# sb-ai-lab/RePlay

Hardware: NVIDIA H100
Metric: sasrec_train_seq_per_s (higher is better)
Workload: dtype bf16

## Files before the change

### replay_b200/csrc/rp_ce_head.cu

```cuda
#include <type_traits>

#include "rp_host.h"
#include "rp_gemm_desc.h"
#include "rp_sm90.cuh"

namespace rp {

static constexpr int kT = 128;
static constexpr int kChunk = 128 * 128;
static constexpr float kLog2e = 1.4426950408889634f;
static constexpr float kLn2 = 0.6931471805599453f;
static constexpr int kThreads = 256;
static constexpr int kTN = 64;

__device__ __forceinline__ float bce_sigmoid(float x, float& one_plus_e) {
  const float e = ex2f(-fabsf(x) * kLog2e);
  one_plus_e = 1.f + e;
  return __fdividef(x >= 0.f ? 1.f : e, one_plus_e);
}
template <int KCH, int NSTAGE, bool BCE = false>
__global__ void __launch_bounds__(kThreads, 1)
ce_fwd_kernel(const __grid_constant__ CUtensorMap tmA, const __grid_constant__ CUtensorMap tmB,
              const int32_t* __restrict__ n_valid_ptr, int n_items, int n_splits, const float* __restrict__ bias,
              float2* __restrict__ part ,
// ... 219 lines not shown
    for (int i = 0; i < (int)gridDim.x; ++i) s += reinterpret_cast<volatile float*>(block_sums)[i];
    loss_out[0] = s * inv_n;
    loss_out[1] = inv_n;
  }
}

struct CeDirect {
  __nv_bfloat16* d_hc;
  float* lse;
  float* cvec;
  float* row_loss;
  CeRowOpts row;
  int use_lse_off;
};

__device__ __forceinline__ float crow_of(const CeDirect& d, int r, int n_valid) {
  return r < n_valid ? (d.use_lse_off ? -d.lse[r] * kLog2e : 0.f) : -INFINITY;
}

__global__ void __launch_bounds__(1024) ce_loss_reduce_kernel(const float* __restrict__ row_loss, const int32_t* __restrict__ n_valid_ptr,
                                                              const int32_t* __restrict__ safe_flag, float* __restrict__ loss_out,
                                                              int run_if_safe) {
  if (safe_flag && (*safe_flag != 0) != (run_if_safe != 0)) return;
  __shared__ float red[1024];
  const int n_valid = *n_valid_ptr;
  float a = 0.f;
  for (int i = threadIdx.x; i < n_valid; i += 1024) a += row_loss[i];
  red[threadIdx.x] = a;
  __syncthreads();
  for (int o = 512; o > 0; o >>= 1) {
    if ((int)threadIdx.x < o) red[threadIdx.x] += red[threadIdx.x + o];
    __syncthreads();
  }
  if (threadIdx.x == 0) {
    const float inv_n = n_valid > 0 ? 1.f / (float)n_valid : 0.f;
    loss_out[0] = red[0] * inv_n;
    loss_out[1] = inv_n;
  }
}

template <int KCH, int NSTAGE, int TN, int MODE, bool HAS_BIAS>
__global__ void __launch_bounds__(kThreads, 1)
ce_bwd_kernel(const __grid_constant__ CUtensorMap tmA, const __grid_constant__ CUtensorMap tmB,
              const __nv_bfloat16* __restrict__ a_rows ,
              const float* __restrict__ cvec , const int32_t* __restrict__ labels,
              const __nv_bfloat16* __restrict__ table, const float* __restrict__ loss_inv ,
              const int32_t* __restrict__ n_valid_ptr, int n_items, const float* __restrict__ bias,
              float* __restrict__ d_bias, void* __restrict__ out, const int32_t* __restrict__ safe_flag, int run_if_safe,
              int n_splits, int capacity, float* __restrict__ zpart, const CeDirect direct) {
  constexpr bool BCE = (MODE >= 3);
  constexpr bool COLCONST = (MODE == 1 || MODE == 4);
  constexpr bool FUSED = (MODE == 2 || MODE == 3);
  constexpr int D = KCH * 64;
  constexpr int kChunkB = TN * 128;
  constexpr int kStage = KCH * kChunkB;
  constexpr int PITCH = D + 4;
  constexpr int kSlots = 2, DW = D / kSlots;
  if (safe_flag && (*safe_flag != 0) != (run_if_safe != 0)) return;
  extern __shared__ __align__(1024) uint8_t smem_raw[];
  uint8_t* smem = reinterpret_cast<uint8_t*>((reinterpret_cast<uintptr_t>(smem_raw) + 1023) & ~uintptr_t(1023));
  uint8_t* sA = smem;
  uint8_t* sB = smem + KCH * kChunk;
  __shared__ float s_row[kT];
  __shared__ float s_dot[kSlots][kT];
  __shared__ uint64_t bar_a, bar_full[NSTAGE];
  __shared__ uint32_t s_released[NSTAGE];

  const int lane = threadIdx.x & 31;
  const int n_valid = *n_valid_ptr;
  const int split = FUSED ? blockIdx.x % n_splits : 0;
  const int n_rows = COLCONST ? n_items : n_valid;
  const int n_cols = COLCONST ? n_valid : n_items;
  const int n_grid = (n_cols + kTN - 1) / kTN;
  const int row_tile = FUSED ? blockIdx.x / n_splits : blockIdx.x;
  const int c_begin = FUSED ? (int)(((long long)n_grid * split) / n_splits) * kTN : 0;
  const int c_end = FUSED ? min(n_cols, (int)(((long long)n_grid * (split + 1)) / n_splits) * kTN) : n_cols;
  const int n_ct = c_end > c_begin ? (c_end - c_begin + TN - 1) / TN : 0;
  const int r0 = row_tile * kT;
  if (r0 >= n_rows) return;

  if (threadIdx.x == 0) {
    mbar_init(&bar_a, 1);
    for (int i = 0; i < NSTAGE; ++i) {
      mbar_init(&bar_full[i], 1);
      s_released[i] = 0;
    }
    fence_barrier_init();
    tma_prefetch_desc(&tmA);
    tma_prefetch_desc(&tmB);
  }
  __syncthreads();
  auto issue = [&](int jl) {
    const uint32_t s = jl % NSTAGE;
    mbar_arrive_expect_tx(&bar_full[s], kStage);
    for (int kc = 0; kc < KCH; ++kc) tma_load_2d(sB + s * kStage + kc * kChunkB, &tmB, &bar_full[s], kc * 64, c_begin + jl * TN);
  };
  if (threadIdx.x == 0) {
    mbar_arrive_expect_tx(&bar_a, KCH * kChunk);
    for (int kc = 0; kc < KCH; ++kc) tma_load_2d(sA + kc * kChunk, &tmA, &bar_a, kc * 64, r0);
    for (int jl = 0; jl < NSTAGE && jl < n_ct; ++jl) issue(jl);
  }
  const int t = threadIdx.x & 127, wg = threadIdx.x >> 7;
  const int fc = frag_col(t);
  const int rla = 64 * wg + frag_row(t), rlb = rla + 8;
  float crow_a = 0.f, crow_b = 0.f;
  if (MODE == 0) {
    crow_a = (r0 + rla < n_valid) ? cvec[r0 + rla] : -INFINITY;
    crow_b = (r0 + rlb < n_valid) ? cvec[r0 + rlb] : -INFINITY;
  }
  if (FUSED && !BCE) {
    crow_a = (r0 + rla < n_valid) ? (direct.use_lse_off ? -direct.lse[r0 + rla] * kLog2e : 0.f) : -INFINITY;
    crow_b = (r0 + rlb < n_valid) ? (direct.use_lse_off ? -direct.lse[r0 + rlb] * kLog2e : 0.f) : -INFINITY;
  }
  float brow_a = 0.f, brow_b = 0.f;
  if (BCE && COLCONST && HAS_BIAS) {
    brow_a = r0 + rla < n_items ? __ldg(bias + r0 + rla) : 0.f;
    brow_b = r0 + rlb < n_items ? __ldg(bias + r0 + rlb) : 0.f;
  }
  float za = 0.f, zb = 0.f;
  float acc[D / 2];
  acc_zero(acc);
  float sacc[TN / 2];
  mbar_wait(&bar_a, 0);
  const uint32_t a_base = smem_u32(sA) + wg * 8192;
  auto issue_s = [&](int jl) {
    mbar_wait(&bar_full[jl % NSTAGE], (jl / NSTAGE) & 1);
    const uint32_t b0 = smem_u32(sB + (jl % NSTAGE) * kStage);
    wg_fence();
#pragma unroll
    for (int kc = 0; kc < KCH; ++kc)
#pragma unroll
      for (int ks = 0; ks < 4; ++ks)
        WgmmaSS<TN>::template run<0, 0>(sacc, desc_k(a_base + kc * kChunk + ks * 32), desc_k(b0 + kc * kChunkB + ks * 32),
                                        (kc | ks) != 0);
    wg_commit();
  };
  constexpr bool kSAhead = MODE != 3;
  if (n_ct > 0) {
    issue_s(0);
    wg_wait<0>();
    wg_fence_acc(sacc);
  }
  if (kSAhead && wg == 1 && n_ct > 0) named_bar_arrive(2, 256);
  for (int jl = 0; jl < n_ct; ++jl) {
    const uint32_t s = jl % NSTAGE;
    const uint32_t b0 = smem_u32(sB + s * kStage);
    const int col0 = c_begin + jl * TN + fc;
    uint32_t pk[TN / 4];
    if constexpr (BCE) {
      float pa = 1.f, pb = 1.f;
#pragma unroll
      for (int q = 0; q < TN / 8; ++q) {
        float g[4];
#pragma unroll
        for (int e = 0; e < 2; ++e) {
          const int col = col0 + 8 * q + e;
          const bool in = col < c_end;
          float va = sacc[4 * q + e], vb = sacc[4 * q + 2 + e];
          if (HAS_BIAS) {
            const float ba = COLCONST ? brow_a : (in ? __ldg(bias + col) : 0.f);
            const float bb = COLCONST ? brow_b : ba;
            va += ba;
// ... 18 lines not shown
        pk[2 * q + 1] = pack_bf16(g[2], g[3]);
      }
      if (FUSED) {
        za += __log2f(pa) * kLn2;
        zb += __log2f(pb) * kLn2;
      }
    } else {
#pragma unroll
      for (int q = 0; q < TN / 8; ++q) {
        float g[4];
#pragma unroll
        for (int e = 0; e < 2; ++e) {
          const int col = col0 + 8 * q + e;
          float va = sacc[4 * q + e], vb = sacc[4 * q + 2 + e];
          if (COLCONST) {
            const float cc = __ldg(cvec + col);
            g[e] = ex2f(fmaf(va, kLog2e, cc));
            g[2 + e] = ex2f(fmaf(vb, kLog2e, cc));
          } else {
            const bool in = col < c_end;
            if (HAS_BIAS && in) {
              const float bb = __ldg(bias + col);
              va += bb;
              vb += bb;
            }
            g[e] = in ? ex2f(fmaf(va, kLog2e, crow_a)) : 0.f;
            g[2 + e] = in ? ex2f(fmaf(vb, kLog2e, crow_b)) : 0.f;
          }
        }
        if (FUSED || (COLCONST && HAS_BIAS)) {
          za += g[0] + g[1];
// ... 1 lines not shown
        }
        pk[2 * q] = pack_bf16(g[0], g[1]);
        pk[2 * q + 1] = pack_bf16(g[2], g[3]);
      }
    }
    if (kSAhead) named_bar_sync(2 + wg, 256);
    wg_fence();
#pragma unroll
    for (int kk = 0; kk < TN / 16; ++kk) {
      const uint32_t af[4] = {pk[4 * kk], pk[4 * kk + 1], pk[4 * kk + 2], pk[4 * kk + 3]};
      WgmmaRS<D>::template run<1>(acc, af, desc_mn(b0 + kk * 2048, kChunkB), 1);
    }
    wg_commit();
    const bool more = jl + 1 < n_ct;
    if constexpr (kSAhead) {
      if (more) issue_s(jl + 1);
      else wg_commit();
      if (wg == 0) named_bar_arrive(3, 256);
      else if (more) named_bar_arrive(2, 256);
      wg_wait<1>();
    } else {
      wg_wait<0>();
    }
    wg_fence_acc(acc);
    __syncwarp();
    if (lane == 0 && jl + NSTAGE < n_ct && smem_count_acq_rel(&s_released[s]) % 8 == 7) {
      fence_proxy_async();
      issue(jl + NSTAGE);
    }
    if (!kSAhead && more) issue_s(jl + 1);
    wg_wait<0>();
    wg_fence_acc(sacc);
  }
#pragma unroll
  for (int o = 1; o <= 2; o <<= 1) {
    za += __shfl_xor_sync(0xffffffffu, za, o);
    zb += __shfl_xor_sync(0xffffffffu, zb, o);
  }
  if (fc == 0) {
    s_row[rla] = za;
    s_row[rlb] = zb;
  }
  named_bar_sync(1, 256);
  float* stage = reinterpret_cast<float*>(sB);
  acc_to_stage(acc, stage, PITCH, 64 * wg, 0);
  named_bar_sync(1, 256);
  const int row = t, slot = wg;
  const int r = r0 + row;
  const float* arow = stage + row * PITCH + slot * DW;
  if constexpr (BCE) {
    const float inv_n = n_valid > 0 ? 1.f / (float)n_valid : 0.f;
    if (COLCONST) {
      if (r < n_items) {
// ... 44 lines not shown
#pragma unroll 4
        for (int c = 0; c < DW; c += 4) dst[c >> 2] = *reinterpret_cast<const float4*>(arow + c);
      }
    }
  } else if (COLCONST) {
    float* o = reinterpret_cast<float*>(out);
    const float rs = (HAS_BIAS && r < n_items) ? __expf(bias[r]) : 1.f;
    if (HAS_BIAS && slot == 0 && r < n_items) d_bias[r] = s_row[row] * rs;
    if (r < n_items) {
      float4* dst = reinterpret_cast<float4*>(o + (size_t)r * D + slot * DW);
#pragma unroll 4
      for (int c = 0; c < DW; c += 4) {
        const float4 v = *reinterpret_cast<const float4*>(arow + c);
        dst[c >> 2] = make_float4(v.x * rs, v.y * rs, v.z * rs, v.w * rs);
      }
    }
  } else if (FUSED && direct.d_hc != nullptr) {
    const float z = s_row[row];
    const bool live = r < n_valid;
    const float inv_n = n_valid > 0 ? 1.f / (float)n_valid : 0.f;
    const int y = live ? labels[r] : 0;
    float wg_ = (live && direct.row.w_ext) ? direct.row.w_ext[r] : 1.f;
    if (direct.row.kind == 1) {
      float dp = 0.f;
      if (live) {
        const uint4* ey = reinterpret_cast<const uint4*>(table + (size_t)y * D + slot * DW);
        const uint4* hr = reinterpret_cast<const uint4*>(a_rows + (size_t)r * D + slot * DW);
#pragma unroll 4
        for (int q = 0; q < DW / 8; ++q) {
          const uint4 e = __ldg(ey + q), hh = __ldg(hr + q);
          const __nv_bfloat162* e2 = reinterpret_cast<const __nv_bfloat162*>(&e);
          const __nv_bfloat162* h2 = reinterpret_cast<const __nv_bfloat162*>(&hh);
#pragma unroll
          for (int pp = 0; pp < 4; ++pp) {
            const float2 ef = __bfloat1622float2(e2[pp]), hf = __bfloat1622float2(h2[pp]);
            dp = fmaf(hf.x, ef.x, fmaf(hf.y, ef.y, dp));
          }
        }
      }
      s_dot[slot][row] = dp;
      named_bar_sync(1, 256);
      float zy0 = s_dot[0][row] + s_dot[1][row];
      if (HAS_BIAS) zy0 += bias[y];
      named_bar_sync(1, 256);
      float rl_unused;
      if (live) ce_row_terms(direct.row, r, __logf(z) - crow_of(direct, r, n_valid) * kLn2, zy0, rl_unused, wg_);
    }
    const float scale = live ? wg_ * inv_n / z : 0.f;
    const float lab = wg_ * inv_n;
    float dot = 0.f;
    if (live) {
      const uint4* ey = reinterpret_cast<const uint4*>(table + (size_t)y * D + slot * DW);
      const uint4* hr = reinterpret_cast<const uint4*>(a_rows + (size_t)r * D + slot * DW);
      uint4* dst = reinterpret_cast<uint4*>(direct.d_hc + (size_t)r * D + slot * DW);
#pragma unroll 4
      for (int q = 0; q < DW / 8; ++q) {
        const uint4 e = __ldg(ey + q), hh = __ldg(hr + q);
        const __nv_bfloat162* e2 = reinterpret_cast<const __nv_bfloat162*>(&e);
        const __nv_bfloat162* h2 = reinterpret_cast<const __nv_bfloat162*>(&hh);
        uint4 w;
        uint32_t* w32 = reinterpret_cast<uint32_t*>(&w);
#pragma unroll
        for (int pp = 0; pp < 4; ++pp) {
          const float2 ef = __bfloat1622float2(e2[pp]), hf = __bfloat1622float2(h2[pp]);
          dot = fmaf(hf.x, ef.x, fmaf(hf.y, ef.y, dot));
          w32[pp] = pack_bf16(arow[8 * q + 2 * pp] * scale - lab * ef.x, arow[8 * q + 2 * pp + 1] * scale - lab * ef.y);
        }
        dst[q] = w;
      }
    }
    s_dot[slot][row] = dot;
    named_bar_sync(1, 256);
    if (slot == 0 && r < capacity) {
      if (live) {
        float zy = s_dot[0][row] + s_dot[1][row];
        if (HAS_BIAS) zy += bias[y];
        const float lse2 = log2f(z) - crow_of(direct, r, n_valid);
        float rl, wg2;
        ce_row_terms(direct.row, r, lse2 * kLn2, zy, rl, wg2);
        direct.lse[r] = lse2 * kLn2;
        direct.cvec[r] = -lse2 + log2f(wg2 * inv_n);
        direct.row_loss[r] = rl;
        if (direct.row.roww) direct.row.roww[r] = wg2;
      } else {
        direct.cvec[r] = -INFINITY;
      }
    }
  } else if (FUSED) {
    float* o = reinterpret_cast<float*>(out) + (size_t)split * capacity * D;
    if (r < n_valid) {
      if (slot == 0) zpart[(size_t)split * capacity + r] = s_row[row];
      float4* dst = reinterpret_cast<float4*>(o + (size_t)r * D + slot * DW);
#pragma unroll 4
      for (int c = 0; c < DW; c += 4) dst[c >> 2] = *reinterpret_cast<const float4*>(arow + c);
    }
  } else {
    __nv_bfloat16* o = reinterpret_cast<__nv_bfloat16*>(out);
    if (r < n_valid) {
      const float inv_n = loss_inv[0] * (direct.row.roww ? direct.row.roww[r] : 1.f);
      const int y = labels[r];
      const uint4* ey = reinterpret_cast<const uint4*>(table + (size_t)y * D + slot * DW);
      uint4* dst = reinterpret_cast<uint4*>(o + (size_t)r * D + slot * DW);
#pragma unroll 4
      for (int q = 0; q < DW / 8; ++q) {
        const uint4 e = ey[q];
        const __nv_bfloat162* e2 = reinterpret_cast<const __nv_bfloat162*>(&e);
        uint4 w;
        uint32_t* w32 = reinterpret_cast<uint32_t*>(&w);
#pragma unroll
// ... 75 lines not shown
    me = fmaxf(me, __shfl_xor_sync(0xffffffffu, me, o));
    mb = fmaxf(mb, __shfl_xor_sync(0xffffffffu, mb, o));
  }
  if (lane == 0) {
    atomicMax(bound + 0, __float_as_uint(mh));
    atomicMax(bound + 1, __float_as_uint(me));
    atomicMax(bound + 2, __float_as_uint(mb));
  }
}

__global__ void ce_flag_kernel(const unsigned int* __restrict__ bound, int32_t* __restrict__ safe_flag) {
  const float b = sqrtf(__uint_as_float(bound[0]) * __uint_as_float(bound[1])) + __uint_as_float(bound[2]);
  *safe_flag = (b * kLog2e < 100.f) ? 1 : 0;
}

__global__ void ce_fused_finalize_kernel(const float* __restrict__ part_dh, const float* __restrict__ zpart,
                                         const __nv_bfloat16* __restrict__ hc, const __nv_bfloat16* __restrict__ table,
                                         const int32_t* __restrict__ labels, const float* __restrict__ bias,
                                         const int32_t* __restrict__ n_valid_ptr, const int32_t* __restrict__ safe_flag,
                                         int n_splits, int z_slots, int capacity, int d, float* __restrict__ lse_out,
                                         float* __restrict__ cvec, __nv_bfloat16* __restrict__ d_hc,
                                         float* __restrict__ block_sums, unsigned int* __restrict__ ticket,
                                         float* __restrict__ loss_out, const CeRowOpts row, int use_lse_off, int run_if_safe) {
  if ((*safe_flag != 0) != (run_if_safe != 0)) return;
  const int n_valid = *n_valid_ptr;
  const float inv_n = n_valid > 0 ? 1.f / (float)n_valid : 0.f;
  const int lane = threadIdx.x & 31, wpb = blockDim.x >> 5;
  float local = 0.f;
  for (int t = blockIdx.x * wpb + (threadIdx.x >> 5); t < capacity; t += gridDim.x * wpb) {
    if (t >= n_valid) {
      if (lane == 0) cvec[t] = -INFINITY;
      continue;
    }
    float z = 0.f;
    for (int i = lane; i < n_splits * z_slots; i += 32) z += zpart[(size_t)i * capacity + t];
#pragma unroll
    for (int o = 16; o > 0; o >>= 1) z += __shfl_xor_sync(0xffffffffu, z, o);
    const int y = labels[t];
    const __nv_bfloat16* hr = hc + (size_t)t * d;
    const __nv_bfloat16* er = table + (size_t)y * d;
    float dot = 0.f;
    for (int c = lane * 4; c < d; c += 128) {
      const uint2 hraw = *reinterpret_cast<const uint2*>(hr + c), eraw = *reinterpret_cast<const uint2*>(er + c);
      const float2 h0 = __bfloat1622float2(*reinterpret_cast<const __nv_bfloat162*>(&hraw.x));
      const float2 h1 = __bfloat1622float2(*reinterpret_cast<const __nv_bfloat162*>(&hraw.y));
      const float2 e0 = __bfloat1622float2(*reinterpret_cast<const __nv_bfloat162*>(&eraw.x));
      const float2 e1 = __bfloat1622float2(*reinterpret_cast<const __nv_bfloat162*>(&eraw.y));
      dot = fmaf(h0.x, e0.x, fmaf(h0.y, e0.y, fmaf(h1.x, e1.x, fmaf(h1.y, e1.y, dot))));
    }
#pragma unroll
    for (int o = 16; o > 0; o >>= 1) dot += __shfl_xor_sync(0xffffffffu, dot, o);
    if (bias) dot += bias[y];
    const float lse2 = log2f(z) + (use_lse_off ? lse_out[t] * kLog2e : 0.f);
    float rl, wg;
    ce_row_terms(row, t, lse2 * kLn2, dot, rl, wg);
    const float scale = wg * inv_n / z, lab = wg * inv_n;
    for (int c = lane * 4; c < d; c += 128) {
      const uint2 eraw = *reinterpret_cast<const uint2*>(er + c);
      const float2 e0 = __bfloat1622float2(*reinterpret_cast<const __nv_bfloat162*>(&eraw.x));
      const float2 e1 = __bfloat1622float2(*reinterpret_cast<const __nv_bfloat162*>(&eraw.y));
      float4 a = make_float4(0.f, 0.f, 0.f, 0.f);
#pragma unroll 8
      for (int p = 0; p < n_splits; ++p) {
        const float4 v = __ldg(reinterpret_cast<const float4*>(part_dh + ((size_t)p * capacity + t) * d + c));
        a.x += v.x; a.y += v.y; a.z += v.z; a.w += v.w;
      }
      uint2 o;
      o.x = pack_bf16(a.x * scale - lab * e0.x, a.y * scale - lab * e0.y);
      o.y = pack_bf16(a.z * scale - lab * e1.x, a.w * scale - lab * e1.y);
      *reinterpret_cast<uint2*>(d_hc + (size_t)t * d + c) = o;
    }
    if (lane == 0) {
      lse_out[t] = lse2 * kLn2;
      cvec[t] = -lse2 + log2f(wg * inv_n);
      if (row.roww) row.roww[t] = wg;
      local += rl;
    }
  }
  __shared__ float red[32];
  __shared__ bool last;
  if (lane == 0) red[threadIdx.x >> 5] = local;
  __syncthreads();
  if (threadIdx.x == 0) {
    float sum = 0.f;
    for (int i = 0; i < wpb; ++i) sum += red[i];
    block_sums[blockIdx.x] = sum;
    __threadfence();
    last = (atomicAdd(ticket, 1u) == gridDim.x - 1);
  }
  __syncthreads();
  if (last && threadIdx.x == 0) {
    __threadfence();
    float sum = 0.f;
    for (int i = 0; i < (int)gridDim.x; ++i) sum += reinterpret_cast<volatile float*>(block_sums)[i];
    loss_out[0] = sum * inv_n;
    loss_out[1] = inv_n;
  }
}

__global__ void ce_dh_reduce_kernel(const float* __restrict__ part, int n_splits, long long split_stride, int rows, int c0,
                                    __nv_bfloat16* __restrict__ d_hc, const __nv_bfloat16* __restrict__ table,
                                    const int32_t* __restrict__ labels, const float* __restrict__ loss_inv,
                                    const int32_t* __restrict__ n_valid_ptr, int d, const float* __restrict__ roww) {
  const int n_valid = *n_valid_ptr;
  const int lane = threadIdx.x & 31, wpb = blockDim.x >> 5;
  for (int r = blockIdx.x * wpb + (threadIdx.x >> 5); r < rows && c0 + r < n_valid; r += gridDim.x * wpb) {
    const int t = c0 + r;
    const float inv_n = loss_inv[0] * (roww ? roww[t] : 1.f);
    const __nv_bfloat16* e = table + (size_t)labels[t] * d;
    for (int c = lane * 4; c < d; c += 128) {
      float4 a = make_float4(0.f, 0.f, 0.f, 0.f);
// ... 164 lines not shown
  }
  return best;
}

}

using namespace rp;

struct CeWs {
  float2* part; float* block_sums; unsigned int* ticket; unsigned int* bound; int32_t* flag; float* zpart; float* roww; float* part_dh;
};
static const int kMaxSplits = 8;
static const int kMaxSplitsFwd = 32;
static const int kWideSplitK = 16;

static size_t ce_ws_base_bytes(int cap, int d) {
  return (size_t)cap * kMaxSplitsFwd * 2 * sizeof(float2) + 4096 + 64 + (size_t)kMaxSplits * cap * 4 +
         (size_t)(cap + 3) / 4 * 16 + (d <= 256 ? (size_t)kMaxSplits * cap * d * 4 : 0) + 256;
}
static size_t ce_ws_bytes(int cap, int n_items, int d) {
  size_t b = (ce_ws_base_bytes(cap, d) + 1023) / 1024 * 1024;
  if (d > 256) {
    const size_t rows = (size_t)wide_chunk_rows(cap, n_items);
    b += rows * wide_ldg(n_items) * 2;
    b += (size_t)kWideSplitK * rows * d * 4;
  }
  return b;
}
static CeWs ce_ws(void* workspace, int cap, int d) {
  uint8_t* w = reinterpret_cast<uint8_t*>(workspace);
  CeWs r;
  r.part = reinterpret_cast<float2*>(w);
  w += (size_t)cap * kMaxSplitsFwd * 2 * sizeof(float2);
// ... 76 lines not shown
                             const int32_t* n_valid, const float* bias, float* part_dh, int grid, int n_splits, int capacity,
                             float* zpart, cudaStream_t stream, const CeDirect& direct) {
  switch (d) {
    case 64:
      return launch_ce_bwd<1, 8, 128, 3>(tmA, table, n_items, hc, nullptr, labels, table, nullptr, n_valid, n_items, bias, nullptr,
                                         part_dh, grid, nullptr, 0, n_splits, capacity, zpart, stream, direct);
    case 128:
      return launch_ce_bwd<2, 8, 64, 3>(tmA, table, n_items, hc, nullptr, labels, table, nullptr, n_valid, n_items, bias, nullptr,
                                        part_dh, grid, nullptr, 0, n_splits, capacity, zpart, stream, direct);
    case 256:
      return launch_ce_bwd<4, 4, 64, 3>(tmA, table, n_items, hc, nullptr, labels, table, nullptr, n_valid, n_items, bias, nullptr,
                                        part_dh, grid, nullptr, 0, n_splits, capacity, zpart, stream, direct);
    default:
      return RP_ESHAPE;
  }
}

RP_API int rp_ce_head_fwd_w(const void* hc, const void* table, const float* bias, const int32_t* labels,
                            const int32_t* n_valid, int capacity, int n_items, int d, float* loss_out, float* lse, float* cvec,
                            void* d_hc, int n_valid_hint, const float* row_weight, int loss_kind, float log_eps, float clamp,
                            void* workspace, size_t workspace_bytes, void* stream_);
RP_API int rp_ce_head_fwd(const void* hc, const void* table, const float* bias, const int32_t* labels,
                          const int32_t* n_valid, int capacity, int n_items, int d, float* loss_out, float* lse, float* cvec,
                          void* d_hc, int n_valid_hint, void* workspace, size_t workspace_bytes, void* stream_) {
  return rp_ce_head_fwd_w(hc, table, bias, labels, n_valid, capacity, n_items, d, loss_out, lse, cvec, d_hc, n_valid_hint, nullptr,
                          0, 0.f, 0.f, workspace, workspace_bytes, stream_);
}

RP_API int rp_ce_head_fwd_w(const void* hc, const void* table, const float* bias, const int32_t* labels,
                            const int32_t* n_valid, int capacity, int n_items, int d, float* loss_out, float* lse, float* cvec,
// ... 12 lines not shown
  CUtensorMap tmA, tmB;
  int rc;
  if ((rc = make_tmap_bf16(&tmA, hc, capacity, d, d, 128)) != RP_OK) return rc;
  if ((rc = make_tmap_bf16(&tmB, table, n_items, d, d, 128)) != RP_OK) return rc;
  RP_CUDA_CHECK(cudaMemsetAsync(ws.ticket, 0, 64, stream));
  const int32_t* skip = nullptr;
  int blocks = (capacity + 7) / 8;
  if (blocks > 1024) blocks = 1024;
  if (fused) {
    ce_bound_kernel<<<sm_count() * 8, 256, 0, stream>>>(reinterpret_cast<const __nv_bfloat16*>(hc),
                                                        reinterpret_cast<const __nv_bfloat16*>(table), bias, n_valid, n_items, d,
                                                        ws.bound);
    RP_LAUNCH_CHECK();
    ce_flag_kernel<<<1, 1, 0, stream>>>(ws.bound, ws.flag);
    RP_LAUNCH_CHECK();
    const int P = pick_splits(hint_tiles, n_item_tiles);
    CeDirect direct{nullptr, lse, nullptr, nullptr, CeRowOpts{row_weight, ws.roww, loss_kind, log_eps, clamp}, 0};
    if (P == 1) {
      direct.d_hc = reinterpret_cast<__nv_bfloat16*>(d_hc);
      direct.cvec = cvec;
      direct.row_loss = ws.zpart;
    }
    rc = dispatch_ce_bwd<2>(d, tmA, table, n_items, hc, cvec, labels, table, loss_out + 1, n_valid, n_items, bias, nullptr, ws.part_dh,
                            n_tok_tiles * P, ws.flag, 1, P, capacity, ws.zpart, stream, direct);
    if (rc != RP_OK) return rc;
    if (P == 1) {
      ce_loss_reduce_kernel<<<1, 1024, 0, stream>>>(ws.zpart, n_valid, ws.flag, loss_out, 1);
      RP_LAUNCH_CHECK();
    } else
    ce_fused_finalize_kernel<<<blocks, 256, 0, stream>>>(ws.part_dh, ws.zpart, reinterpret_cast<const __nv_bfloat16*>(hc),
                                                         reinterpret_cast<const __nv_bfloat16*>(table), labels, bias, n_valid,
                                                         ws.flag, P, 1, capacity, d, lse, cvec,
                                                         reinterpret_cast<__nv_bfloat16*>(d_hc), ws.block_sums, ws.ticket, loss_out,
                                                         CeRowOpts{row_weight, ws.roww, loss_kind, log_eps, clamp}, 0, 1);
    RP_LAUNCH_CHECK();
    skip = ws.flag;
  }
  int P2 = pick_splits(hint_tiles, n_item_tiles, kMaxSplitsFwd);
  if (fused) {
    const int cap = (2 * sm_count() + n_tok_tiles - 1) / n_tok_tiles;
    if (P2 > cap) P2 = cap;
  }
  switch (d) {
    case 64: rc = launch_ce_fwd<1, 8>(tmA, tmB, n_valid, n_items, P2, n_tok_tiles, bias, ws.part, skip, stream); break;
    case 128: rc = launch_ce_fwd<2, 8>(tmA, tmB, n_valid, n_items, P2, n_tok_tiles, bias, ws.part, skip, stream); break;
    case 256: rc = launch_ce_fwd<4, 8>(tmA, tmB, n_valid, n_items, P2, n_tok_tiles, bias, ws.part, skip, stream); break;
    default: rc = launch_ce_fwd<8, 5>(tmA, tmB, n_valid, n_items, P2, n_tok_tiles, bias, ws.part, skip, stream); break;
  }
  if (rc != RP_OK) return rc;
  ce_finalize_kernel<<<blocks, 256, 0, stream>>>(ws.part, reinterpret_cast<const __nv_bfloat16*>(hc),
                                                 reinterpret_cast<const __nv_bfloat16*>(table), labels, bias, n_valid, P2,
                                                 capacity, d, lse, cvec, ws.block_sums, ws.ticket, loss_out, skip,
                                                 CeRowOpts{row_weight, ws.roww, loss_kind, log_eps, clamp});
  RP_LAUNCH_CHECK();
  if (fused) {
    const int P = pick_splits(hint_tiles, n_item_tiles);
    CeDirect direct{nullptr, lse, nullptr, nullptr, CeRowOpts{row_weight, ws.roww, loss_kind, log_eps, clamp}, 1};
    if (P == 1) {
      direct.d_hc = reinterpret_cast<__nv_bfloat16*>(d_hc);
      direct.cvec = cvec;
      direct.row_loss = ws.zpart;
    }
    RP_CUDA_CHECK(cudaMemsetAsync(ws.ticket, 0, 4, stream));
    rc = dispatch_ce_bwd<2>(d, tmA, table, n_items, hc, cvec, labels, table, loss_out + 1, n_valid, n_items, bias, nullptr, ws.part_dh,
                            n_tok_tiles * P, ws.flag, 0, P, capacity, ws.zpart, stream, direct);
    if (rc != RP_OK) return rc;
    if (P == 1) {
      ce_loss_reduce_kernel<<<1, 1024, 0, stream>>>(ws.zpart, n_valid, ws.flag, loss_out, 0);
    } else {
      ce_fused_finalize_kernel<<<blocks, 256, 0, stream>>>(ws.part_dh, ws.zpart, reinterpret_cast<const __nv_bfloat16*>(hc),
                                                           reinterpret_cast<const __nv_bfloat16*>(table), labels, bias, n_valid,
                                                           ws.flag, P, 1, capacity, d, lse, cvec,
                                                           reinterpret_cast<__nv_bfloat16*>(d_hc), ws.block_sums, ws.ticket, loss_out,
                                                           CeRowOpts{row_weight, ws.roww, loss_kind, log_eps, clamp}, 1, 0);
    }
    RP_LAUNCH_CHECK();
  }
  return RP_OK;
}

RP_API int rp_ce_head_bwd(const void* hc, const void* table, const float* bias, const int32_t* labels,
                          const int32_t* n_valid, int capacity, int n_items, int d, const float* loss_out ,
                          const float* cvec , void* d_hc, float* d_table, float* d_bias, int fused,
                          int n_valid_hint, void* workspace, size_t workspace_bytes, void* stream_) {
  cudaStream_t stream = reinterpret_cast<cudaStream_t>(stream_);
  if (!hc || !table || !labels || !n_valid || !loss_out || !cvec || !d_hc || !d_table) return RP_EINVAL;
  if ((bias == nullptr) != (d_bias == nullptr)) return RP_EINVAL;
  if (capacity <= 0 || n_items <= 0) return RP_ESHAPE;
  if (d != 64 && d != 128 && d != 256 && d != 512) return RP_ESHAPE;
  if ((fused || d == 512) && (!workspace || workspace_bytes < ce_ws_bytes(capacity, n_items, d))) return RP_EWORKSPACE;
  const float* roww = (workspace && workspace_bytes >= ce_ws_bytes(capacity, n_items, d)) ? ce_ws(workspace, capacity, d).roww : nullptr;
// ... 228 lines not shown
```

Baseline: 81120.

## Make fused CE backward persistent with stream-K work split across SMs

Replaces the row-tile × column-split grid of the fused CE backward kernel with a persistent grid of one CTA per SM. Each CTA takes a contiguous range of (row tile, column tile) units and can span several row tiles, reloading the A tile between segments. Row tiles a CTA covers whole are finalized in-kernel. Row tiles split across CTAs write partials to per-CTA slots, which a new straddle finalize kernel combines. The aim is better load balance and less wave quantization; the cost is more complex indexing and an extra finalize launch. It also prefetches the column constants into registers for MODE 1.

```diff
diff --git a/replay_b200/csrc/rp_ce_head.cu b/replay_b200/csrc/rp_ce_head.cu
--- a/replay_b200/csrc/rp_ce_head.cu
+++ b/replay_b200/csrc/rp_ce_head.cu
@@ -257,10 +257,6 @@
   int use_lse_off;
 };
 
-__device__ __forceinline__ float crow_of(const CeDirect& d, int r, int n_valid) {
-  return r < n_valid ? (d.use_lse_off ? -d.lse[r] * kLog2e : 0.f) : -INFINITY;
-}
-
 __global__ void __launch_bounds__(1024) ce_loss_reduce_kernel(const float* __restrict__ row_loss, const int32_t* __restrict__ n_valid_ptr,
                                                               const int32_t* __restrict__ safe_flag, float* __restrict__ loss_out,
                                                               int run_if_safe) {
@@ -282,6 +278,14 @@
   }
 }
 
+__device__ __forceinline__ long long fused_range_start(int b, int n_ctas, int n_rt, int n_grid) {
+  const long long n_units = (long long)n_rt * n_grid;
+  if (n_rt >= n_ctas) return n_units * b / n_ctas;
+  const int P = n_ctas / max(n_rt, 1);
+  if (b >= n_rt * P) return n_units;
+  return (long long)(b / P) * n_grid + (long long)n_grid * (b % P) / P;
+}
+
 template <int KCH, int NSTAGE, int TN, int MODE, bool HAS_BIAS>
 __global__ void __launch_bounds__(kThreads, 1)
 ce_bwd_kernel(const __grid_constant__ CUtensorMap tmA, const __grid_constant__ CUtensorMap tmB,
@@ -294,6 +298,7 @@
   constexpr bool BCE = (MODE >= 3);
   constexpr bool COLCONST = (MODE == 1 || MODE == 4);
   constexpr bool FUSED = (MODE == 2 || MODE == 3);
+  constexpr bool PERSIST = (MODE == 2);
   constexpr int D = KCH * 64;
   constexpr int kChunkB = TN * 128;
   constexpr int kStage = KCH * kChunkB;
@@ -311,16 +316,37 @@
 
   const int lane = threadIdx.x & 31;
   const int n_valid = *n_valid_ptr;
-  const int split = FUSED ? blockIdx.x % n_splits : 0;
+  const int split = (FUSED && !PERSIST) ? blockIdx.x % n_splits : 0;
   const int n_rows = COLCONST ? n_items : n_valid;
   const int n_cols = COLCONST ? n_valid : n_items;
   const int n_grid = (n_cols + kTN - 1) / kTN;
-  const int row_tile = FUSED ? blockIdx.x / n_splits : blockIdx.x;
-  const int c_begin = FUSED ? (int)(((long long)n_grid * split) / n_splits) * kTN : 0;
-  const int c_end = FUSED ? min(n_cols, (int)(((long long)n_grid * (split + 1)) / n_splits) * kTN) : n_cols;
-  const int n_ct = c_end > c_begin ? (c_end - c_begin + TN - 1) / TN : 0;
-  const int r0 = row_tile * kT;
-  if (r0 >= n_rows) return;
+  int row_tile, n_seg = 1, c_begin0, c_end_last;
+  if constexpr (PERSIST) {
+    const int n_rt = (n_rows + kT - 1) / kT;
+    const long long u0 = fused_range_start(blockIdx.x, gridDim.x, n_rt, n_grid);
+    const long long u1 = fused_range_start(blockIdx.x + 1, gridDim.x, n_rt, n_grid);
+    if (u0 >= u1) return;
+    row_tile = (int)(u0 / n_grid);
+    const int r_last = (int)((u1 - 1) / n_grid);
+    n_seg = r_last - row_tile + 1;
+    c_begin0 = (int)(u0 - (long long)row_tile * n_grid) * kTN;
+    c_end_last = min(n_cols, (int)(u1 - (long long)r_last * n_grid) * kTN);
+  } else {
+    row_tile = FUSED ? blockIdx.x / n_splits : blockIdx.x;
+    c_begin0 = FUSED ? (int)(((long long)n_grid * split) / n_splits) * kTN : 0;
+    c_end_last = FUSED ? min(n_cols, (int)(((long long)n_grid * (split + 1)) / n_splits) * kTN) : n_cols;
+    if (row_tile * kT >= n_rows) return;
+  }
+  auto seg_begin = [&](int k) { return k == 0 ? c_begin0 : 0; };
+  auto seg_end = [&](int k) { return k == n_seg - 1 ? c_end_last : n_cols; };
+  auto n_tiles = [](int b, int e) { return e > b ? (e - b + TN - 1) / TN : 0; };
+  const int n_ct0 = n_tiles(c_begin0, seg_end(0)), n_ct_full = n_tiles(0, n_cols);
+  const int n_ct_total = n_seg == 1 ? n_ct0 : n_ct0 + (n_seg - 2) * n_ct_full + n_tiles(0, c_end_last);
+  auto tile_col = [&](int g) {
+    if (g < n_ct0) return c_begin0 + g * TN;
+    const int k = 1 + (g - n_ct0) / n_ct_full;
+    return (k < n_seg - 1 ? g : g - n_ct0) % n_ct_full * TN;
+  };
 
   if (threadIdx.x == 0) {
     mbar_init(&bar_a, 1);
@@ -333,42 +359,44 @@
     tma_prefetch_desc(&tmB);
   }
   __syncthreads();
-  auto issue = [&](int jl) {
-    const uint32_t s = jl % NSTAGE;
+  auto issue = [&](int g) {
+    const uint32_t s = g % NSTAGE;
+    const int c = tile_col(g);
     mbar_arrive_expect_tx(&bar_full[s], kStage);
-    for (int kc = 0; kc < KCH; ++kc) tma_load_2d(sB + s * kStage + kc * kChunkB, &tmB, &bar_full[s], kc * 64, c_begin + jl * TN);
+    for (int kc = 0; kc < KCH; ++kc) tma_load_2d(sB + s * kStage + kc * kChunkB, &tmB, &bar_full[s], kc * 64, c);
+  };
+  auto load_a = [&](int r0) {
+    mbar_arrive_expect_tx(&bar_a, KCH * kChunk);
+    for (int kc = 0; kc < KCH; ++kc) tma_load_2d(sA + kc * kChunk, &tmA, &bar_a, kc * 64, r0);
   };
   if (threadIdx.x == 0) {
-    mbar_arrive_expect_tx(&bar_a, KCH * kChunk);
-    for (int kc = 0; kc < KCH; ++kc) tma_load_2d(sA + kc * kChunk, &tmA, &bar_a, kc * 64, r0);
-    for (int jl = 0; jl < NSTAGE && jl < n_ct; ++jl) issue(jl);
+    load_a(row_tile * kT);
+    for (int g = 0; g < NSTAGE && g < n_ct_total; ++g) issue(g);
   }
   const int t = threadIdx.x & 127, wg = threadIdx.x >> 7;
   const int fc = frag_col(t);
   const int rla = 64 * wg + frag_row(t), rlb = rla + 8;
-  float crow_a = 0.f, crow_b = 0.f;
-  if (MODE == 0) {
-    crow_a = (r0 + rla < n_valid) ? cvec[r0 + rla] : -INFINITY;
-    crow_b = (r0 + rlb < n_valid) ? cvec[r0 + rlb] : -INFINITY;
-  }
-  if (FUSED && !BCE) {
-    crow_a = (r0 + rla < n_valid) ? (direct.use_lse_off ? -direct.lse[r0 + rla] * kLog2e : 0.f) : -INFINITY;
-    crow_b = (r0 + rlb < n_valid) ? (direct.use_lse_off ? -direct.lse[r0 + rlb] * kLog2e : 0.f) : -INFINITY;
-  }
   float brow_a = 0.f, brow_b = 0.f;
   if (BCE && COLCONST && HAS_BIAS) {
+    const int r0 = row_tile * kT;
     brow_a = r0 + rla < n_items ? __ldg(bias + r0 + rla) : 0.f;
     brow_b = r0 + rlb < n_items ? __ldg(bias + r0 + rlb) : 0.f;
   }
-  float za = 0.f, zb = 0.f;
+  float za, zb;
   float acc[D / 2];
-  acc_zero(acc);
   float sacc[TN / 2];
-  mbar_wait(&bar_a, 0);
+  constexpr bool kPreC = (MODE == 1);
+  float2 coff[kPreC ? TN / 8 : 1];
+  auto load_c = [&](int col0) {
+    if constexpr (kPreC) {
+#pragma unroll
+      for (int q = 0; q < TN / 8; ++q) coff[q] = __ldg(reinterpret_cast<const float2*>(cvec + col0 + 8 * q));
+    }
+  };
   const uint32_t a_base = smem_u32(sA) + wg * 8192;
-  auto issue_s = [&](int jl) {
-    mbar_wait(&bar_full[jl % NSTAGE], (jl / NSTAGE) & 1);
-    const uint32_t b0 = smem_u32(sB + (jl % NSTAGE) * kStage);
+  auto issue_s = [&](int g) {
+    mbar_wait(&bar_full[g % NSTAGE], (g / NSTAGE) & 1);
+    const uint32_t b0 = smem_u32(sB + (g % NSTAGE) * kStage);
     wg_fence();
 #pragma unroll
     for (int kc = 0; kc < KCH; ++kc)
@@ -379,16 +407,91 @@
     wg_commit();
   };
   constexpr bool kSAhead = MODE != 3;
+  int r0 = row_tile * kT, c_begin = 0, c_end = 0;
+  auto fused_rows_out = [&](int k, float crow_a, float crow_b) {
+    const float inv_n = n_valid > 0 ? 1.f / (float)n_valid : 0.f;
+    const bool whole = c_begin == 0 && c_end == n_cols;
+    const int slot = 2 * blockIdx.x + (k == 0 ? 0 : 1);
+#pragma unroll
+    for (int h = 0; h < 2; ++h) {
+      const int rl = h ? rlb : rla, r = r0 + rl;
+      const float z = h ? zb : za;
+      if (!whole) {
+        float* o = reinterpret_cast<float*>(out) + ((size_t)slot * kT + rl) * D + fc;
+#pragma unroll
+        for (int j = 0; j < D / 8; ++j) *reinterpret_cast<float2*>(o + 8 * j) = make_float2(acc[4 * j + 2 * h], acc[4 * j + 2 * h + 1]);
+        if (fc == 0) zpart[slot * kT + rl] = z;
+        continue;
+      }
+      const bool live = r < n_valid;
+      const int y = live ? labels[r] : 0;
+      const __nv_bfloat16* ey = table + (size_t)y * D + fc;
+      const __nv_bfloat16* hr = a_rows + (size_t)r * D + fc;
+      float dot = 0.f;
+      if (live) {
+#pragma unroll
+        for (int j = 0; j < D / 8; ++j) {
+          const float2 ef = __bfloat1622float2(__ldg(reinterpret_cast<const __nv_bfloat162*>(ey + 8 * j)));
+          const float2 hf = __bfloat1622float2(__ldg(reinterpret_cast<const __nv_bfloat162*>(hr + 8 * j)));
+          dot = fmaf(hf.x, ef.x, fmaf(hf.y, ef.y, dot));
+        }
+      }
+      dot = quad_sum(dot);
+      if (HAS_BIAS && live) dot += bias[y];
+      const float lse2 = log2f(z) - (h ? crow_b : crow_a);
+      float rl_loss = 0.f, wgt = 0.f;
+      if (live) ce_row_terms(direct.row, r, lse2 * kLn2, dot, rl_loss, wgt);
+      const float scale = live ? wgt * inv_n / z : 0.f, lab = wgt * inv_n;
+      if (live) {
+        uint32_t* dst = reinterpret_cast<uint32_t*>(direct.d_hc + (size_t)r * D + fc);
+#pragma unroll
+        for (int j = 0; j < D / 8; ++j) {
+          const float2 ef = __bfloat1622float2(__ldg(reinterpret_cast<const __nv_bfloat162*>(ey + 8 * j)));
+          dst[4 * j] = pack_bf16(acc[4 * j + 2 * h] * scale - lab * ef.x, acc[4 * j + 2 * h + 1] * scale - lab * ef.y);
+        }
+      }
+      if (fc == 0 && r < capacity) {
+        if (live) {
+          direct.lse[r] = lse2 * kLn2;
+          direct.cvec[r] = -lse2 + log2f(wgt * inv_n);
+          direct.row_loss[r] = rl_loss;
+          if (direct.row.roww) direct.row.roww[r] = wgt;
+        } else {
+          direct.cvec[r] = -INFINITY;
+        }
+      }
+    }
+  };
+  for (int k = 0, g0 = 0; k < n_seg; ++k) {
+  r0 = (row_tile + k) * kT;
+  c_begin = seg_begin(k);
+  c_end = seg_end(k);
+  const int n_ct = n_tiles(c_begin, c_end);
+  float crow_a = 0.f, crow_b = 0.f;
+  if (MODE == 0) {
+    crow_a = (r0 + rla < n_valid) ? cvec[r0 + rla] : -INFINITY;
+    crow_b = (r0 + rlb < n_valid) ? cvec[r0 + rlb] : -INFINITY;
+  }
+  if (FUSED && !BCE) {
+    crow_a = (r0 + rla < n_valid) ? (direct.use_lse_off ? -direct.lse[r0 + rla] * kLog2e : 0.f) : -INFINITY;
+    crow_b = (r0 + rlb < n_valid) ? (direct.use_lse_off ? -direct.lse[r0 + rlb] * kLog2e : 0.f) : -INFINITY;
+  }
+  za = 0.f;
+  zb = 0.f;
+  acc_zero(acc);
+  mbar_wait(&bar_a, k & 1);
   if (n_ct > 0) {
-    issue_s(0);
+    issue_s(g0);
+    load_c(tile_col(g0) + fc);
     wg_wait<0>();
     wg_fence_acc(sacc);
   }
   if (kSAhead && wg == 1 && n_ct > 0) named_bar_arrive(2, 256);
   for (int jl = 0; jl < n_ct; ++jl) {
-    const uint32_t s = jl % NSTAGE;
+    const int g = g0 + jl;
+    const uint32_t s = g % NSTAGE;
     const uint32_t b0 = smem_u32(sB + s * kStage);
-    const int col0 = c_begin + jl * TN + fc;
+    const int col0 = tile_col(g) + fc;
     uint32_t pk[TN / 4];
     if constexpr (BCE) {
       float pa = 1.f, pb = 1.f;
@@ -437,7 +540,7 @@
           const int col = col0 + 8 * q + e;
           float va = sacc[4 * q + e], vb = sacc[4 * q + 2 + e];
           if (COLCONST) {
-            const float cc = __ldg(cvec + col);
+            const float cc = e ? coff[q].y : coff[q].x;
             g[e] = ex2f(fmaf(va, kLog2e, cc));
             g[2 + e] = ex2f(fmaf(vb, kLog2e, cc));
           } else {
@@ -469,8 +572,12 @@
     wg_commit();
     const bool more = jl + 1 < n_ct;
     if constexpr (kSAhead) {
-      if (more) issue_s(jl + 1);
-      else wg_commit();
+      if (more) {
+        issue_s(g + 1);
+        load_c(tile_col(g + 1) + fc);
+      } else {
+        wg_commit();
+      }
       if (wg == 0) named_bar_arrive(3, 256);
       else if (more) named_bar_arrive(2, 256);
       wg_wait<1>();
@@ -479,19 +586,27 @@
     }
     wg_fence_acc(acc);
     __syncwarp();
-    if (lane == 0 && jl + NSTAGE < n_ct && smem_count_acq_rel(&s_released[s]) % 8 == 7) {
+    if (lane == 0 && g + NSTAGE < n_ct_total && smem_count_acq_rel(&s_released[s]) % 8 == 7) {
       fence_proxy_async();
-      issue(jl + NSTAGE);
-    }
-    if (!kSAhead && more) issue_s(jl + 1);
+      issue(g + NSTAGE);
+    }
+    if (!kSAhead && more) issue_s(g + 1);
     wg_wait<0>();
     wg_fence_acc(sacc);
   }
-#pragma unroll
-  for (int o = 1; o <= 2; o <<= 1) {
-    za += __shfl_xor_sync(0xffffffffu, za, o);
-    zb += __shfl_xor_sync(0xffffffffu, zb, o);
-  }
+  g0 += n_ct;
+  za = quad_sum(za);
+  zb = quad_sum(zb);
+  if constexpr (PERSIST) {
+    named_bar_sync(1, 256);
+    if (threadIdx.x == 0 && k + 1 < n_seg) {
+      fence_proxy_async();
+      load_a(r0 + kT);
+    }
+    fused_rows_out(k, crow_a, crow_b);
+  }
+  }
+  if constexpr (PERSIST) return;
   if (fc == 0) {
     s_row[rla] = za;
     s_row[rlb] = zb;
@@ -566,85 +681,6 @@
         const float4 v = *reinterpret_cast<const float4*>(arow + c);
         dst[c >> 2] = make_float4(v.x * rs, v.y * rs, v.z * rs, v.w * rs);
       }
-    }
-  } else if (FUSED && direct.d_hc != nullptr) {
-    const float z = s_row[row];
-    const bool live = r < n_valid;
-    const float inv_n = n_valid > 0 ? 1.f / (float)n_valid : 0.f;
-    const int y = live ? labels[r] : 0;
-    float wg_ = (live && direct.row.w_ext) ? direct.row.w_ext[r] : 1.f;
-    if (direct.row.kind == 1) {
-      float dp = 0.f;
-      if (live) {
-        const uint4* ey = reinterpret_cast<const uint4*>(table + (size_t)y * D + slot * DW);
-        const uint4* hr = reinterpret_cast<const uint4*>(a_rows + (size_t)r * D + slot * DW);
-#pragma unroll 4
-        for (int q = 0; q < DW / 8; ++q) {
-          const uint4 e = __ldg(ey + q), hh = __ldg(hr + q);
-          const __nv_bfloat162* e2 = reinterpret_cast<const __nv_bfloat162*>(&e);
-          const __nv_bfloat162* h2 = reinterpret_cast<const __nv_bfloat162*>(&hh);
-#pragma unroll
-          for (int pp = 0; pp < 4; ++pp) {
-            const float2 ef = __bfloat1622float2(e2[pp]), hf = __bfloat1622float2(h2[pp]);
-            dp = fmaf(hf.x, ef.x, fmaf(hf.y, ef.y, dp));
-          }
-        }
-      }
-      s_dot[slot][row] = dp;
-      named_bar_sync(1, 256);
-      float zy0 = s_dot[0][row] + s_dot[1][row];
-      if (HAS_BIAS) zy0 += bias[y];
-      named_bar_sync(1, 256);
-      float rl_unused;
-      if (live) ce_row_terms(direct.row, r, __logf(z) - crow_of(direct, r, n_valid) * kLn2, zy0, rl_unused, wg_);
-    }
-    const float scale = live ? wg_ * inv_n / z : 0.f;
-    const float lab = wg_ * inv_n;
-    float dot = 0.f;
-    if (live) {
-      const uint4* ey = reinterpret_cast<const uint4*>(table + (size_t)y * D + slot * DW);
-      const uint4* hr = reinterpret_cast<const uint4*>(a_rows + (size_t)r * D + slot * DW);
-      uint4* dst = reinterpret_cast<uint4*>(direct.d_hc + (size_t)r * D + slot * DW);
-#pragma unroll 4
-      for (int q = 0; q < DW / 8; ++q) {
-        const uint4 e = __ldg(ey + q), hh = __ldg(hr + q);
-        const __nv_bfloat162* e2 = reinterpret_cast<const __nv_bfloat162*>(&e);
-        const __nv_bfloat162* h2 = reinterpret_cast<const __nv_bfloat162*>(&hh);
-        uint4 w;
-        uint32_t* w32 = reinterpret_cast<uint32_t*>(&w);
-#pragma unroll
-        for (int pp = 0; pp < 4; ++pp) {
-          const float2 ef = __bfloat1622float2(e2[pp]), hf = __bfloat1622float2(h2[pp]);
-          dot = fmaf(hf.x, ef.x, fmaf(hf.y, ef.y, dot));
-          w32[pp] = pack_bf16(arow[8 * q + 2 * pp] * scale - lab * ef.x, arow[8 * q + 2 * pp + 1] * scale - lab * ef.y);
-        }
-        dst[q] = w;
-      }
-    }
-    s_dot[slot][row] = dot;
-    named_bar_sync(1, 256);
-    if (slot == 0 && r < capacity) {
-      if (live) {
-        float zy = s_dot[0][row] + s_dot[1][row];
-        if (HAS_BIAS) zy += bias[y];
-        const float lse2 = log2f(z) - crow_of(direct, r, n_valid);
-        float rl, wg2;
-        ce_row_terms(direct.row, r, lse2 * kLn2, zy, rl, wg2);
-        direct.lse[r] = lse2 * kLn2;
-        direct.cvec[r] = -lse2 + log2f(wg2 * inv_n);
-        direct.row_loss[r] = rl;
-        if (direct.row.roww) direct.row.roww[r] = wg2;
-      } else {
-        direct.cvec[r] = -INFINITY;
-      }
-    }
-  } else if (FUSED) {
-    float* o = reinterpret_cast<float*>(out) + (size_t)split * capacity * D;
-    if (r < n_valid) {
-      if (slot == 0) zpart[(size_t)split * capacity + r] = s_row[row];
-      float4* dst = reinterpret_cast<float4*>(o + (size_t)r * D + slot * DW);
-#pragma unroll 4
-      for (int c = 0; c < DW; c += 4) dst[c >> 2] = *reinterpret_cast<const float4*>(arow + c);
     }
   } else {
     __nv_bfloat16* o = reinterpret_cast<__nv_bfloat16*>(out);
@@ -750,28 +786,38 @@
   *safe_flag = (b * kLog2e < 100.f) ? 1 : 0;
 }
 
-__global__ void ce_fused_finalize_kernel(const float* __restrict__ part_dh, const float* __restrict__ zpart,
-                                         const __nv_bfloat16* __restrict__ hc, const __nv_bfloat16* __restrict__ table,
-                                         const int32_t* __restrict__ labels, const float* __restrict__ bias,
-                                         const int32_t* __restrict__ n_valid_ptr, const int32_t* __restrict__ safe_flag,
-                                         int n_splits, int z_slots, int capacity, int d, float* __restrict__ lse_out,
-                                         float* __restrict__ cvec, __nv_bfloat16* __restrict__ d_hc,
-                                         float* __restrict__ block_sums, unsigned int* __restrict__ ticket,
-                                         float* __restrict__ loss_out, const CeRowOpts row, int use_lse_off, int run_if_safe) {
+static constexpr int kFinBlocks = 8;
+__global__ void ce_straddle_finalize_kernel(const float* __restrict__ part_dh, const float* __restrict__ zpart,
+                                            const __nv_bfloat16* __restrict__ hc, const __nv_bfloat16* __restrict__ table,
+                                            const int32_t* __restrict__ labels, const float* __restrict__ bias,
+                                            const int32_t* __restrict__ n_valid_ptr, const int32_t* __restrict__ safe_flag,
+                                            int run_if_safe, int n_ctas, int n_items, int capacity, int d,
+                                            float* __restrict__ lse_out, float* __restrict__ cvec, __nv_bfloat16* __restrict__ d_hc,
+                                            float* __restrict__ row_loss, const CeRowOpts row, int use_lse_off) {
   if ((*safe_flag != 0) != (run_if_safe != 0)) return;
   const int n_valid = *n_valid_ptr;
+  const int n_grid = (n_items + kTN - 1) / kTN;
+  const int n_rt = (n_valid + kT - 1) / kT;
+  const long long n_units = (long long)n_rt * n_grid;
+  auto start = [&](int c) { return fused_range_start(c, n_ctas, n_rt, n_grid); };
+  const int b = blockIdx.x / kFinBlocks, part = blockIdx.x % kFinBlocks;
+  if (b == 0 || start(b) >= n_units || start(b) % n_grid == 0) return;
+  const int rt = (int)(start(b) / n_grid);
+  const long long u_lo = (long long)rt * n_grid, u_hi = min(n_units, u_lo + n_grid);
+  if (start(b - 1) > u_lo) return;
+  int c_hi = b;
+  while (c_hi + 1 < n_ctas && start(c_hi + 1) < u_hi) ++c_hi;
   const float inv_n = n_valid > 0 ? 1.f / (float)n_valid : 0.f;
   const int lane = threadIdx.x & 31, wpb = blockDim.x >> 5;
-  float local = 0.f;
-  for (int t = blockIdx.x * wpb + (threadIdx.x >> 5); t < capacity; t += gridDim.x * wpb) {
+  for (int i = part * (kT / kFinBlocks) + (threadIdx.x >> 5); i < (part + 1) * (kT / kFinBlocks); i += wpb) {
+    const int t = rt * kT + i;
     if (t >= n_valid) {
-      if (lane == 0) cvec[t] = -INFINITY;
+      if (lane == 0 && t < capacity) cvec[t] = -INFINITY;
       continue;
     }
     float z = 0.f;
-    for (int i = lane; i < n_splits * z_slots; i += 32) z += zpart[(size_t)i * capacity + t];
-#pragma unroll
-    for (int o = 16; o > 0; o >>= 1) z += __shfl_xor_sync(0xffffffffu, z, o);
+    for (int c = b - 1; c <= c_hi; ++c)
+      if (start(c) < start(c + 1)) z += zpart[(size_t)(2 * c + (start(c) >= u_lo ? 0 : 1)) * kT + i];
     const int y = labels[t];
     const __nv_bfloat16* hr = hc + (size_t)t * d;
     const __nv_bfloat16* er = table + (size_t)y * d;
@@ -796,9 +842,10 @@
       const float2 e0 = __bfloat1622float2(*reinterpret_cast<const __nv_bfloat162*>(&eraw.x));
       const float2 e1 = __bfloat1622float2(*reinterpret_cast<const __nv_bfloat162*>(&eraw.y));
       float4 a = make_float4(0.f, 0.f, 0.f, 0.f);
-#pragma unroll 8
-      for (int p = 0; p < n_splits; ++p) {
-        const float4 v = __ldg(reinterpret_cast<const float4*>(part_dh + ((size_t)p * capacity + t) * d + c));
+      for (int cc = b - 1; cc <= c_hi; ++cc) {
+        if (start(cc) == start(cc + 1)) continue;
+        const size_t slot = 2 * cc + (start(cc) >= u_lo ? 0 : 1);
+        const float4 v = __ldg(reinterpret_cast<const float4*>(part_dh + (slot * kT + i) * d + c));
         a.x += v.x; a.y += v.y; a.z += v.z; a.w += v.w;
       }
       uint2 o;
@@ -810,27 +857,8 @@
       lse_out[t] = lse2 * kLn2;
       cvec[t] = -lse2 + log2f(wg * inv_n);
       if (row.roww) row.roww[t] = wg;
-      local += rl;
-    }
-  }
-  __shared__ float red[32];
-  __shared__ bool last;
-  if (lane == 0) red[threadIdx.x >> 5] = local;
-  __syncthreads();
-  if (threadIdx.x == 0) {
-    float sum = 0.f;
-    for (int i = 0; i < wpb; ++i) sum += red[i];
-    block_sums[blockIdx.x] = sum;
-    __threadfence();
-    last = (atomicAdd(ticket, 1u) == gridDim.x - 1);
-  }
-  __syncthreads();
-  if (last && threadIdx.x == 0) {
-    __threadfence();
-    float sum = 0.f;
-    for (int i = 0; i < (int)gridDim.x; ++i) sum += reinterpret_cast<volatile float*>(block_sums)[i];
-    loss_out[0] = sum * inv_n;
-    loss_out[1] = inv_n;
+      row_loss[t] = rl;
+    }
   }
 }
 
@@ -1025,9 +1053,15 @@
 static const int kMaxSplitsFwd = 32;
 static const int kWideSplitK = 16;
 
+static size_t ce_fused_slots() { return 2 * (size_t)sm_count(); }
+static size_t ce_part_floats(int cap, int d) {
+  if (d > 256) return 0;
+  const size_t bce = (size_t)kMaxSplits * cap * d, ce = ce_fused_slots() * kT * (d + 1);
+  return bce > ce ? bce : ce;
+}
 static size_t ce_ws_base_bytes(int cap, int d) {
   return (size_t)cap * kMaxSplitsFwd * 2 * sizeof(float2) + 4096 + 64 + (size_t)kMaxSplits * cap * 4 +
-         (size_t)(cap + 3) / 4 * 16 + (d <= 256 ? (size_t)kMaxSplits * cap * d * 4 : 0) + 256;
+         (size_t)(cap + 3) / 4 * 16 + ce_part_floats(cap, d) * 4 + 256;
 }
 static size_t ce_ws_bytes(int cap, int n_items, int d) {
   size_t b = (ce_ws_base_bytes(cap, d) + 1023) / 1024 * 1024;
@@ -1134,6 +1168,25 @@
     default:
       return RP_ESHAPE;
   }
+}
+
+static int ce_fused_pass(int d, const CUtensorMap& tmA, const void* hc, const void* table, const float* bias,
+                         const int32_t* labels, const int32_t* n_valid, int capacity, int n_items, float* loss_out, float* lse,
+                         float* cvec, void* d_hc, const CeRowOpts& row, const CeWs& ws, int after_two_pass, cudaStream_t stream) {
+  const int grid = sm_count(), run_if_safe = !after_two_pass;
+  float* zp = ws.part_dh + ce_fused_slots() * kT * d;
+  const CeDirect direct{reinterpret_cast<__nv_bfloat16*>(d_hc), lse, cvec, ws.zpart , row, after_two_pass};
+  int rc = dispatch_ce_bwd<2>(d, tmA, table, n_items, hc, cvec, labels, table, loss_out + 1, n_valid, n_items, bias, nullptr,
+                              ws.part_dh, grid, ws.flag, run_if_safe, 1, capacity, zp, stream, direct);
+  if (rc != RP_OK) return rc;
+  ce_straddle_finalize_kernel<<<grid * kFinBlocks, 256, 0, stream>>>(ws.part_dh, zp, reinterpret_cast<const __nv_bfloat16*>(hc),
+                                                        reinterpret_cast<const __nv_bfloat16*>(table), labels, bias, n_valid,
+                                                        ws.flag, run_if_safe, grid, n_items, capacity, d, lse, cvec,
+                                                        reinterpret_cast<__nv_bfloat16*>(d_hc), ws.zpart, row, after_two_pass);
+  RP_LAUNCH_CHECK();
+  ce_loss_reduce_kernel<<<1, 1024, 0, stream>>>(ws.zpart, n_valid, ws.flag, loss_out, run_if_safe);
+  RP_LAUNCH_CHECK();
+  return RP_OK;
 }
 
 RP_API int rp_ce_head_fwd_w(const void* hc, const void* table, const float* bias, const int32_t* labels,
@@ -1176,26 +1229,9 @@
     RP_LAUNCH_CHECK();
     ce_flag_kernel<<<1, 1, 0, stream>>>(ws.bound, ws.flag);
     RP_LAUNCH_CHECK();
-    const int P = pick_splits(hint_tiles, n_item_tiles);
-    CeDirect direct{nullptr, lse, nullptr, nullptr, CeRowOpts{row_weight, ws.roww, loss_kind, log_eps, clamp}, 0};
-    if (P == 1) {
-      direct.d_hc = reinterpret_cast<__nv_bfloat16*>(d_hc);
-      direct.cvec = cvec;
-      direct.row_loss = ws.zpart;
-    }
-    rc = dispatch_ce_bwd<2>(d, tmA, table, n_items, hc, cvec, labels, table, loss_out + 1, n_valid, n_items, bias, nullptr, ws.part_dh,
-                            n_tok_tiles * P, ws.flag, 1, P, capacity, ws.zpart, stream, direct);
+    rc = ce_fused_pass(d, tmA, hc, table, bias, labels, n_valid, capacity, n_items, loss_out, lse, cvec, d_hc,
+                       CeRowOpts{row_weight, ws.roww, loss_kind, log_eps, clamp}, ws, 0, stream);
     if (rc != RP_OK) return rc;
-    if (P == 1) {
-      ce_loss_reduce_kernel<<<1, 1024, 0, stream>>>(ws.zpart, n_valid, ws.flag, loss_out, 1);
-      RP_LAUNCH_CHECK();
-    } else
-    ce_fused_finalize_kernel<<<blocks, 256, 0, stream>>>(ws.part_dh, ws.zpart, reinterpret_cast<const __nv_bfloat16*>(hc),
-                                                         reinterpret_cast<const __nv_bfloat16*>(table), labels, bias, n_valid,
-                                                         ws.flag, P, 1, capacity, d, lse, cvec,
-                                                         reinterpret_cast<__nv_bfloat16*>(d_hc), ws.block_sums, ws.ticket, loss_out,
-                                                         CeRowOpts{row_weight, ws.roww, loss_kind, log_eps, clamp}, 0, 1);
-    RP_LAUNCH_CHECK();
     skip = ws.flag;
   }
   int P2 = pick_splits(hint_tiles, n_item_tiles, kMaxSplitsFwd);
@@ -1216,27 +1252,9 @@
                                                  CeRowOpts{row_weight, ws.roww, loss_kind, log_eps, clamp});
   RP_LAUNCH_CHECK();
   if (fused) {
-    const int P = pick_splits(hint_tiles, n_item_tiles);
-    CeDirect direct{nullptr, lse, nullptr, nullptr, CeRowOpts{row_weight, ws.roww, loss_kind, log_eps, clamp}, 1};
-    if (P == 1) {
-      direct.d_hc = reinterpret_cast<__nv_bfloat16*>(d_hc);
-      direct.cvec = cvec;
-      direct.row_loss = ws.zpart;
-    }
-    RP_CUDA_CHECK(cudaMemsetAsync(ws.ticket, 0, 4, stream));
-    rc = dispatch_ce_bwd<2>(d, tmA, table, n_items, hc, cvec, labels, table, loss_out + 1, n_valid, n_items, bias, nullptr, ws.part_dh,
-                            n_tok_tiles * P, ws.flag, 0, P, capacity, ws.zpart, stream, direct);
+    rc = ce_fused_pass(d, tmA, hc, table, bias, labels, n_valid, capacity, n_items, loss_out, lse, cvec, d_hc,
+                       CeRowOpts{row_weight, ws.roww, loss_kind, log_eps, clamp}, ws, 1, stream);
     if (rc != RP_OK) return rc;
-    if (P == 1) {
-      ce_loss_reduce_kernel<<<1, 1024, 0, stream>>>(ws.zpart, n_valid, ws.flag, loss_out, 0);
-    } else {
-      ce_fused_finalize_kernel<<<blocks, 256, 0, stream>>>(ws.part_dh, ws.zpart, reinterpret_cast<const __nv_bfloat16*>(hc),
-                                                           reinterpret_cast<const __nv_bfloat16*>(table), labels, bias, n_valid,
-                                                           ws.flag, P, 1, capacity, d, lse, cvec,
-                                                           reinterpret_cast<__nv_bfloat16*>(d_hc), ws.block_sums, ws.ticket, loss_out,
-                                                           CeRowOpts{row_weight, ws.roww, loss_kind, log_eps, clamp}, 1, 0);
-    }
-    RP_LAUNCH_CHECK();
   }
   return RP_OK;
 }
```

New measurement: 82800, median of 6. 2.1% higher.
